# YxZhxn/Ray3D

Measured on AMD Instinct MI355X. Metric: lifted poses/sec (17-joint, 243-frame window), higher is better.
Workload: dtype f32; 1 GPU; BASELINE configs[1]: synthetic 17-joint 243-frame windows, batch 256 per GPU, forward-only pos+trj (C=256, latent 256, stage 3, camera embedding); batch_per_gpu=256, receptive_field=243, joints=17, parallelism=dp1 (independent window batches, no data-path collective), clock_settle_steps=60, world_size_observed=1

## Files before the change

ray3d_amd/csrc/r3d_tiles.hpp:

```cpp
#pragma once
#include <hip/hip_runtime.h>

#include <algorithm>
#include <type_traits>

#include "r3d_internal.hpp"

namespace r3d {

#ifndef R3D_TS
#define R3D_TS 0
#endif
#ifdef R3D_TIMING
#define R3D_TSTAMP(slot) do { if (dbg && threadIdx.x == 0) dbg[slot] = wall_clock64(); } while (0)
#else
#define R3D_TSTAMP(slot) do { } while (0)
#endif

typedef float f32x16 __attribute__((ext_vector_type(16)));
typedef float f32x4 __attribute__((ext_vector_type(4)));

#define R3D_AS1 __attribute__((address_space(1)))
__device__ __forceinline__ f32x4 gload4(const float *p) { return *(const R3D_AS1 f32x4 *)p; }
__device__ __forceinline__ float gload1(const float *p) { return *(const R3D_AS1 float *)p; }
__device__ __forceinline__ void gstore1(float *p, float v) { *(R3D_AS1 float *)p = v; }
constexpr int ACT_AUX = 16;
typedef unsigned u32x4 __attribute__((ext_vector_type(4)));
typedef unsigned R3D_AS1 *gu32;
struct LateWait { int dw, ndep; gu32 cnt, abort_flag; long long spin_ticks; };
__device__ __forceinline__ void wait_deps_reg(const int dw, const int ndep, const gu32 cnt, const gu32 abort_flag, const long long spin_ticks);
__device__ __forceinline__ __amdgpu_buffer_rsrc_t act_rsrc(const float *base) {
    return __builtin_amdgcn_make_buffer_rsrc(const_cast<float *>(base), 0, 0x7fffffff, 0x00020000);
}
__device__ __forceinline__ f32x4 act_load4(__amdgpu_buffer_rsrc_t r, int byte_off) {
    return __builtin_bit_cast(f32x4, __builtin_amdgcn_raw_buffer_load_b128(r, byte_off, 0, ACT_AUX));
}
__device__ __forceinline__ float act_load1(__amdgpu_buffer_rsrc_t r, int byte_off) {
    return __builtin_bit_cast(float, __builtin_amdgcn_raw_buffer_load_b32(r, byte_off, 0, ACT_AUX));
}
__device__ __forceinline__ void act_store4(__amdgpu_buffer_rsrc_t r, int byte_off, f32x4 v) {
    __builtin_amdgcn_raw_buffer_store_b128(__builtin_bit_cast(u32x4, v), r, byte_off, 0, ACT_AUX);
}
__device__ __forceinline__ void act_store1(__amdgpu_buffer_rsrc_t r, int byte_off, float v) {
    __builtin_amdgcn_raw_buffer_store_b32(__builtin_bit_cast(unsigned, v), r, byte_off, 0, ACT_AUX);
}
__device__ __forceinline__ void tile_drain() { asm volatile("s_waitcnt vmcnt(0)" ::: "memory"); }
__device__ __forceinline__ void tile_signal(const gu32 cnt, const int sig_base, const int sig_add, const int units) {
    int t = threadIdx.x;
    asm volatile("" : "+v"(t));
    if (t < units) __hip_atomic_fetch_add(cnt + sig_base + t, (unsigned)sig_add, __ATOMIC_RELAXED, __HIP_MEMORY_SCOPE_AGENT);
}
__device__ __forceinline__ void tile_signal2(const gu32 cnt, const int base0, const int add0, const int base1, const int add1) {
    int t = threadIdx.x;
    asm volatile("" : "+v"(t));
    if (t < 2) __hip_atomic_fetch_add(cnt + (t == 0 ? base0 : base1), (unsigned)(t == 0 ? add0 : add1), __ATOMIC_RELAXED, __HIP_MEMORY_SCOPE_AGENT);
}
__device__ __forceinline__ float lrelu(const float v, const float slope) { return __builtin_fmaxf(v, v * slope); }


constexpr int LDS_LD = BK + 4;
constexpr int GEMM_THREADS = 512;
constexpr int GEMM_BN = 256;
constexpr int GEMM_MAX_MI = 6;
constexpr int GEMM_STAGES = 3;
constexpr int STAGE_FLOATS = GEMM_MAX_MI * 32 * LDS_LD;
constexpr int LUT_LDS_INTS = 1152;
constexpr int RING_LDS_BYTES = GEMM_STAGES * STAGE_FLOATS * 4;
constexpr int GEMM_LDS_BYTES = 157952;
static_assert(GEMM_LDS_BYTES >= RING_LDS_BYTES, "the ring and the intermediate tile share the allocation");

typedef const LaunchArgs __attribute__((address_space(4))) *LaunchArgsPtr;
typedef const GemmProb __attribute__((address_space(4))) &ProbRef;

constexpr int EPI_LD = GEMM_BN + 4;

constexpr unsigned ACT_SENTINEL_BITS = 0x7fc5a1e7u;
__device__ __forceinline__ float act_canon(const float v) {
    return __builtin_bit_cast(unsigned, v) == ACT_SENTINEL_BITS ? __builtin_bit_cast(float, 0x7fc00000u) : v;
}

template <int MI, int KS>
__device__ __forceinline__ void store_tile(ProbRef P, const f32x16 (&acc)[MI], const int row0, const int col0, float *lds,
                                           const bool second = false) {
    constexpr int COLS = GEMM_BN / KS, WN = 8 / KS;
    constexpr int TPR = COLS / 4;
    constexpr int RPP = GEMM_THREADS / TPR;
    int tid = threadIdx.x;
    asm volatile("" : "+v"(tid));
    const int lane = tid & 63, wave = tid >> 6, li = lane & 31, lh = lane >> 5;
    const int M = P.M, N = P.N;
    const float slope = second ? P.slope2 : P.slope;
    const float *res = P.res;
    const bool canon = P.canon != 0;
    const int ldc = P.ldc, ldr = P.ldr;
    const __amdgpu_buffer_rsrc_t crs = act_rsrc(P.c + (size_t)row0 * ldc + col0);
    const __amdgpu_buffer_rsrc_t rrs = act_rsrc(res ? res + (size_t)row0 * ldr + col0 : P.c);
    const bool writer = wave < WN;
    const float bias = writer ? gload1((second ? P.bias2 : P.bias) + col0 + wave * 32 + li) : 0.0f;
    float *wr = lds + (4 * lh) * EPI_LD + wave * 32 + li;
    const int rd_row = tid / TPR, rd_c4 = (tid % TPR) * 4;
    const bool vec = (col0 + COLS <= N);
#pragma unroll
    for (int mi = 0; mi < MI; ++mi) {
        __syncthreads();
        if (writer) {
#pragma unroll
            for (int r = 0; r < 16; ++r) {
                float v = acc[mi][r] + bias;
                wr[((r & 3) + 8 * (r >> 2)) * EPI_LD] = lrelu(v, slope);
            }
        }
        __syncthreads();
#pragma unroll
        for (int j = 0; j < 32 / RPP; ++j) {
            const int lr = rd_row + RPP * j;
            const int row = row0 + mi * 32 + lr;
            if (row >= M) continue;
            f32x4 v = *reinterpret_cast<const f32x4 *>(lds + lr * EPI_LD + rd_c4);
            const int col = col0 + rd_c4;
            const int lrow = mi * 32 + lr;
            if (vec) {
                if (res) v += act_load4(rrs, (lrow * ldr + rd_c4) * 4);
                if (canon) {
#pragma unroll
                    for (int e = 0; e < 4; ++e) v[e] = act_canon(v[e]);
                }
                act_store4(crs, (lrow * ldc + rd_c4) * 4, v);
            } else {
#pragma unroll
                for (int e = 0; e < 4; ++e)
                    if (col + e < N) {
                        const float o = v[e] + (res ? act_load1(rrs, (lrow * ldr + rd_c4 + e) * 4) : 0.0f);
                        act_store1(crs, (lrow * ldc + rd_c4 + e) * 4, canon ? act_canon(o) : o);
                    }
            }
        }
    }
    __syncthreads();
}

constexpr int PAIR_LD = GEMM_BN + 4;
constexpr int PAIR_MAX_MI = 4;
template <int MI, int KS, bool PAIR = false>
__device__ __forceinline__ void gemm_tile(ProbRef P, const int row0, const int col0, float *smem, long long *dbg, const LateWait late = LateWait{0, 0, nullptr, nullptr, 0}) {
    static_assert(!PAIR || (KS == 1 && MI <= PAIR_MAX_MI), "fused pairs are whole tiles of at most 128 rows");
    constexpr int SF = STAGE_FLOATS;
    R3D_TSTAMP(0);
    static_assert(KS == 1 || (KS == 2 && MI <= 2) || (KS == 4 && MI == 1), "split-K tiles are small tiles");
    constexpr int WN = 8 / KS;
    constexpr int VR = KS * MI * 32;
    constexpr int NA = (VR + 63) / 64;
    constexpr bool PRE = MI <= 3;
    constexpr bool WD2 = MI <= 4;
    constexpr int AD = WD2 ? 5 : 4;
    int tid = threadIdx.x;
    asm volatile("" : "+v"(tid));
    const int lane = tid & 63, wave = tid >> 6;
    const int li = lane & 31, lh = lane >> 5;
    const int wn = wave % WN;
    const int wk = wave / WN;
    const int M = P.M, K = P.K;
    const int nk32 = K / BK;
    const int nk = (nk32 + KS - 1) / KS;
    const int srow = tid >> 3, a_kq = (tid & 7) * 4;

    const bool multi = P.kend[0] < K;
    int seg_ld = P.lda[0], seg_k0 = 0, seg_end = P.kend[0], seg_i = 0;
// ... 35 lines not shown
    auto commit_a = [&](int stage, const Staged &R) {
        float *s = stage == 0 ? smem + st_off : stage == 1 ? smem + SF + st_off : smem + 2 * SF + st_off;
        {
#pragma unroll
            for (int i = 0; i < NA; ++i) *reinterpret_cast<f32x4 *>(s + i * 64 * LDS_LD) = R.a[i];
        }
    };

    const int wave_u = __builtin_amdgcn_readfirstlane(wave);
    __amdgpu_buffer_rsrc_t wrsrc = __builtin_amdgcn_make_buffer_rsrc(
        const_cast<float *>(P.w + ((size_t)((col0 >> 5) + wave_u % WN) * nk32 + wave_u / WN) * 1024), 0,
        (nk32 - wave_u / WN) * 4096, 0x00020000);
    const int w_voff = lane * 16;
    f32x4 rb[4], rbn[4], rbn2[4];
    auto load_w = [&](int kt, f32x4 (&dst)[4]) {
#pragma unroll
        for (int q = 0; q < 4; ++q)
            dst[q] = __builtin_bit_cast(f32x4, __builtin_amdgcn_raw_buffer_load_b128(
                wrsrc, w_voff + q * 1024, kt * KS * 4096, 0));
    };

    f32x16 acc[MI];
#pragma unroll
    for (int mi = 0; mi < MI; ++mi)
#pragma unroll
        for (int r = 0; r < 16; ++r) acc[mi][r] = 0.0f;

    const int a_frag = (wk * MI * 32 + li) * LDS_LD + lh * 16;
    f32x4 av0[PRE ? MI : 1];

    const int last = nk - 1;
    load_w(0, rb);
    if (WD2) load_w(1 < last ? 1 : last, rbn);
    if (late.ndep > 0) wait_deps_reg(late.dw, late.ndep, late.cnt, late.abort_flag, late.spin_ticks);
    {
        Staged r0, r1;
        issue_a(0, r0);
        prep_seg(1 < last ? 1 : last);
        issue_a(1 < last ? 1 : last, r1);
        prep_seg(2 < last ? 2 : last);
        issue_a(2 < last ? 2 : last, ra);
        prep_seg(3 < last ? 3 : last);
        issue_a(3 < last ? 3 : last, ra2);
        prep_seg(4 < last ? 4 : last);
        if (WD2) {
            issue_a(4 < last ? 4 : last, ra3);
            prep_seg(5 < last ? 5 : last);
        }
        if (P.kend[0] < BK) {
            const int width = P.kend[0];
#pragma unroll
            for (int i = 0; i < NA; ++i)
#pragma unroll
                for (int e = 0; e < 4; ++e)
                    if (a_kq + e >= width) r0.a[i][e] = 0.0f;
        }
        commit_a(0, r0);
        commit_a(1, r1);
    }
    __syncthreads();
    if (PRE) {
#pragma unroll
        for (int mi = 0; mi < MI; ++mi) av0[mi] = *reinterpret_cast<const f32x4 *>(smem + a_frag + mi * 32 * LDS_LD);
    }
    R3D_TSTAMP(1);
    int st_cur = 0;
    auto k_tile = [&](int kt, f32x4 (&w_use)[4], f32x4 (&w_load)[4], Staged &stg) {
        const int st_next = st_cur == 2 ? 0 : st_cur + 1, st_next2 = st_next == 2 ? 0 : st_next + 1;
        const float *s = smem + st_cur * SF + a_frag;
        const bool active = KS == 1 || kt * KS + wave_u / WN < nk32;
        auto mfma_q = [&](int q) {
            if (!active) return;
            f32x4 av[MI];
#pragma unroll
            for (int mi = 0; mi < MI; ++mi) {
                if (PRE && q == 0) av[mi] = av0[mi];
                else av[mi] = *reinterpret_cast<const f32x4 *>(s + mi * 32 * LDS_LD + q * 4);
            }
#pragma unroll
            for (int kk = 0; kk < 4; ++kk)
#pragma unroll
                for (int mi = 0; mi < MI; ++mi)
                    acc[mi] = __builtin_amdgcn_mfma_f32_32x32x2f32(av[mi][kk], w_use[q][kk], acc[mi], 0, 0, 0);
        };
        constexpr bool INTERLEAVE = MI >= 3;
        if (!INTERLEAVE) {
            commit_a(st_next2, stg);
            load_w(kt + (WD2 ? 2 : 1) < last ? kt + (WD2 ? 2 : 1) : last, w_load);
            issue_a(kt + AD < last ? kt + AD : last, stg);
            prep_seg(kt + AD + 1 < last ? kt + AD + 1 : last);
        }
        mfma_q(0);
        if (INTERLEAVE) {
            commit_a(st_next2, stg);
            load_w(kt + (WD2 ? 2 : 1) < last ? kt + (WD2 ? 2 : 1) : last, w_load);
        }
        mfma_q(1);
        if (INTERLEAVE) {
            issue_a(kt + AD < last ? kt + AD : last, stg);
            prep_seg(kt + AD + 1 < last ? kt + AD + 1 : last);
        }
        mfma_q(2);
        mfma_q(3);
        if (PRE) {
            const float *sn = smem + st_next * SF + a_frag;
#pragma unroll
            for (int mi = 0; mi < MI; ++mi) av0[mi] = *reinterpret_cast<const f32x4 *>(sn + mi * 32 * LDS_LD);
        }
        __syncthreads();
        st_cur = st_next;
    };
    int kt = 0;
    if (WD2) {
        for (; kt + 2 < nk; kt += 3) {
            k_tile(kt, rb, rbn2, ra);
            k_tile(kt + 1, rbn, rb, ra2);
            k_tile(kt + 2, rbn2, rbn, ra3);
        }
        if (kt < nk) {
            k_tile(kt, rb, rbn2, ra);
            if (kt + 1 < nk) k_tile(kt + 1, rbn, rb, ra2);
        }
    } else {
        for (; kt + 1 < nk; kt += 2) {
            k_tile(kt, rb, rbn, ra);
            k_tile(kt + 1, rbn, rb, ra2);
        }
        if (kt < nk) k_tile(kt, rb, rbn, ra);
    }

    R3D_TSTAMP(2);
    if (KS > 1) {
        constexpr int PHASE_FLOATS = WN * MI * 16 * 64;
        float *red = smem + ((wn * MI) * 16) * 64 + lane;
        if (wk > 0) {
            float *mine = red + wk * PHASE_FLOATS;
#pragma unroll
            for (int mi = 0; mi < MI; ++mi)
#pragma unroll
                for (int r = 0; r < 16; ++r) mine[(mi * 16 + r) * 64] = acc[mi][r];
        }
        __syncthreads();
        if (wk == 0) {
#pragma unroll
            for (int ph = 1; ph < KS; ++ph)
#pragma unroll
                for (int mi = 0; mi < MI; ++mi)
#pragma unroll
                    for (int r = 0; r < 16; ++r) acc[mi][r] += red[ph * PHASE_FLOATS + (mi * 16 + r) * 64];
        }
    }
    R3D_TSTAMP(3);
    if constexpr (PAIR) {
        const float slope1 = P.slope;
        const float bias1 = gload1(P.bias + wave * 32 + li);
        __syncthreads();
#pragma unroll
        for (int mi = 0; mi < MI; ++mi) {
            float *wr = smem + (mi * 32 + 4 * lh) * PAIR_LD + wave * 32 + li;
#pragma unroll
            for (int r = 0; r < 16; ++r) {
                const float v = acc[mi][r] + bias1;
                wr[((r & 3) + 8 * (r >> 2)) * PAIR_LD] = lrelu(v, slope1);
            }
        }
        __syncthreads();
        const int nk2 = P.K2 / BK;
        __amdgpu_buffer_rsrc_t w2rsrc = __builtin_amdgcn_make_buffer_rsrc(
            const_cast<float *>(P.w2 + ((size_t)wave_u * nk2) * 1024), 0, nk2 * 4096, 0x00020000);
        auto load_w2 = [&](int kt, f32x4 (&dst)[4]) {
#pragma unroll
            for (int q = 0; q < 4; ++q)
                dst[q] = __builtin_bit_cast(f32x4, __builtin_amdgcn_raw_buffer_load_b128(w2rsrc, w_voff + q * 1024, kt * 4096, 0));
        };
#pragma unroll
        for (int mi = 0; mi < MI; ++mi)
#pragma unroll
            for (int r = 0; r < 16; ++r) acc[mi][r] = 0.0f;
        const float *h_frag = smem + li * PAIR_LD + lh * 16;
        const int last2 = nk2 - 1;
        auto k_tile2 = [&](int kt2, f32x4 (&w_use)[4], f32x4 (&w_load)[4]) {
            load_w2(kt2 + 2 < last2 ? kt2 + 2 : last2, w_load);
            __builtin_amdgcn_sched_barrier(0);
            const float *s = h_frag + kt2 * BK;
#pragma unroll
            for (int q = 0; q < 4; ++q) {
                f32x4 av[MI];
#pragma unroll
                for (int mi = 0; mi < MI; ++mi) av[mi] = *reinterpret_cast<const f32x4 *>(s + mi * 32 * PAIR_LD + q * 4);
#pragma unroll
                for (int kk = 0; kk < 4; ++kk)
#pragma unroll
                    for (int mi = 0; mi < MI; ++mi)
                        acc[mi] = __builtin_amdgcn_mfma_f32_32x32x2f32(av[mi][kk], w_use[q][kk], acc[mi], 0, 0, 0);
            }
        };
        load_w2(0, rb);
        load_w2(1 < last2 ? 1 : last2, rbn);
        int kt2 = 0;
        for (; kt2 + 2 < nk2; kt2 += 3) {
            k_tile2(kt2, rb, rbn2);
            k_tile2(kt2 + 1, rbn, rb);
            k_tile2(kt2 + 2, rbn2, rbn);
        }
        if (kt2 < nk2) {
            k_tile2(kt2, rb, rbn2);
            if (kt2 + 1 < nk2) k_tile2(kt2 + 1, rbn, rb);
        }
        store_tile<MI, 1>(P, acc, row0, col0, smem, true);
    } else {
        store_tile<MI, KS>(P, acc, row0, col0, smem);
    }
    R3D_TSTAMP(4);
}

template <int NB>
__device__ __forceinline__ void gemm_tile_nb(ProbRef P, ProbRef P2, const int row0, const int row0b, const int col0, const int n0, float *smem, long long *dbg,
                                             const LateWait late = LateWait{0, 0, nullptr, nullptr, 0}) {
    static_assert(NB >= 4 && NB <= 7, "NB = 8 is gemm_tile<1, 1>");
    constexpr int SF = STAGE_FLOATS;
    constexpr int NX = NB - 4;
    constexpr int AD = 5;
    R3D_TSTAMP(0);
    int tid = threadIdx.x;
    asm volatile("" : "+v"(tid));
    const int lane = tid & 63, wave = tid >> 6;
    const int li = lane & 31, lh = lane >> 5;
    const int wave_u = __builtin_amdgcn_readfirstlane(wave);
    const bool main_w = wave_u < 4;
    const bool two = n0 < NB;
    ProbRef PA = two && !main_w ? P2 : P;
    const int rowA = two && !main_w ? row0b : row0;
    const int M = PA.M, K = P.K;
    const int nk = K / BK;
    const int srow = tid >> 3, a_kq = (tid & 7) * 4;
    const int xg0 = (wave_u - 4) * NX;
    int s_blk[4], s_q[4];
#pragma unroll
    for (int s = 0; s < 4; ++s) {
        const int sc = s < NX ? s : 0;
        s_blk[s] = main_w ? wave_u : (NX > 0 ? 4 + (xg0 + sc) / 4 : wave_u - 4);
        s_q[s] = main_w ? s : (NX > 0 ? (xg0 + sc) & 3 : 0);
    }
    const bool multi = PA.kend[0] < K;
// ... 11 lines not shown
    auto prep_seg = [&](int kt) {
        if (!multi) return;
        while (kt * BK >= seg_end) {
            ++seg_i;
            seg_k0 = seg_end;
            seg_ld = PA.lda[seg_i];
            seg_end = PA.kend[seg_i];
            open_seg();
        }
    };
    f32x4 ra, ra2, ra3;
    auto issue_a = [&](int kt, f32x4 &R) {
        R = __builtin_bit_cast(f32x4, __builtin_amdgcn_raw_buffer_load_b128(arsrc, a_voff, (kt * BK - seg_k0) * 4, ACT_AUX));
    };
    const int st_off = srow * LDS_LD + a_kq;
    auto commit_a = [&](int stage, const f32x4 &R) {
        float *sp = stage == 0 ? smem + st_off : stage == 1 ? smem + SF + st_off : smem + 2 * SF + st_off;
        *reinterpret_cast<f32x4 *>(sp) = R;
    };
    const __amdgpu_buffer_rsrc_t wrsrc0 = __builtin_amdgcn_make_buffer_rsrc(
        const_cast<float *>(P.w + (size_t)(col0 >> 5) * nk * 1024), 0, NB * nk * 4096, 0x00020000);
    const __amdgpu_buffer_rsrc_t wrsrc1 = __builtin_amdgcn_make_buffer_rsrc(const_cast<float *>(P2.w), 0, NB * nk * 4096, 0x00020000);
    const int w_voff = lane * 16;
    __amdgpu_buffer_rsrc_t wrsrc[4];
    int w_soff[4], a_off[4];
#pragma unroll
    for (int s = 0; s < 4; ++s) {
        const bool second = s_blk[s] >= n0;
        wrsrc[s] = second ? wrsrc1 : wrsrc0;
        w_soff[s] = __builtin_amdgcn_readfirstlane(((second ? s_blk[s] - n0 : s_blk[s]) * nk) * 4096 + s_q[s] * 1024);
        a_off[s] = (second ? 32 * LDS_LD : 0) + li * LDS_LD + lh * 16 + s_q[s] * 4;
    }
    const int last = nk - 1;
    auto k_loop = [&](auto ns_tag, auto nacc_tag, f32x16 *acc, const __amdgpu_buffer_rsrc_t (&wrs)[4]) {
        constexpr int NS = decltype(ns_tag)::value, NACC = decltype(nacc_tag)::value;
        constexpr int NSL = NS > 0 ? NS : 1;
        f32x4 rb[NSL], rbn[NSL], rbn2[NSL];
        auto load_w = [&](int kt, f32x4 (&dst)[NSL]) {
            if (NS == 0) return;
#pragma unroll
            for (int s = 0; s < NSL; ++s)
                dst[s] = __builtin_bit_cast(f32x4, __builtin_amdgcn_raw_buffer_load_b128(wrs[s], w_voff, w_soff[s] + kt * 4096, 0));
        };
        load_w(0, rb);
        load_w(1 < last ? 1 : last, rbn);
        if (late.ndep > 0) wait_deps_reg(late.dw, late.ndep, late.cnt, late.abort_flag, late.spin_ticks);
        {
            f32x4 r0, r1;
            issue_a(0, r0);
            prep_seg(1 < last ? 1 : last);
            issue_a(1 < last ? 1 : last, r1);
            prep_seg(2 < last ? 2 : last);
            issue_a(2 < last ? 2 : last, ra);
            prep_seg(3 < last ? 3 : last);
            issue_a(3 < last ? 3 : last, ra2);
            prep_seg(4 < last ? 4 : last);
            issue_a(4 < last ? 4 : last, ra3);
            prep_seg(5 < last ? 5 : last);
            commit_a(0, r0);
            commit_a(1, r1);
        }
        __syncthreads();
        f32x4 av0 = *reinterpret_cast<const f32x4 *>(smem + a_off[0]);
        R3D_TSTAMP(1);
        int st_cur = 0;
        auto k_tile = [&](int kt, f32x4 (&w_use)[NSL], f32x4 (&w_load)[NSL], f32x4 &stg) {
            const int st_next = st_cur == 2 ? 0 : st_cur + 1, st_next2 = st_next == 2 ? 0 : st_next + 1;
            const float *sp = smem + st_cur * SF;
            commit_a(st_next2, stg);
            load_w(kt + 2 < last ? kt + 2 : last, w_load);
            issue_a(kt + AD < last ? kt + AD : last, stg);
            prep_seg(kt + AD + 1 < last ? kt + AD + 1 : last);
#pragma unroll
            for (int s = 0; s < NS; ++s) {
                const f32x4 av = s == 0 ? av0 : *reinterpret_cast<const f32x4 *>(sp + a_off[s]);
#pragma unroll
                for (int kk = 0; kk < 4; ++kk)
                    acc[s % NACC] = __builtin_amdgcn_mfma_f32_32x32x2f32(av[kk], w_use[s][kk], acc[s % NACC], 0, 0, 0);
            }
            if (NS > 0) av0 = *reinterpret_cast<const f32x4 *>(smem + st_next * SF + a_off[0]);
            __syncthreads();
            st_cur = st_next;
        };
        int kt = 0;
        for (; kt + 2 < nk; kt += 3) {
            k_tile(kt, rb, rbn2, ra);
            k_tile(kt + 1, rbn, rb, ra2);
            k_tile(kt + 2, rbn2, rbn, ra3);
        }
        if (kt < nk) {
            k_tile(kt, rb, rbn2, ra);
            if (kt + 1 < nk) k_tile(kt + 1, rbn, rb, ra2);
        }
    };
    constexpr int PART = 16 * 64;
    f32x16 fin;
    if (main_w) {
        f32x16 acc[1];
#pragma unroll
        for (int r = 0; r < 16; ++r) acc[0][r] = 0.0f;
        const __amdgpu_buffer_rsrc_t wm[4] = {wrsrc[0], wrsrc[0], wrsrc[0], wrsrc[0]};
        k_loop(std::integral_constant<int, 4>{}, std::integral_constant<int, 1>{}, acc, wm);
        fin = acc[0];
        R3D_TSTAMP(2);
        if (NX > 0) __syncthreads();
    } else {
        constexpr int NA_ = NX > 0 ? NX : 1;
        f32x16 acc[NA_];
#pragma unroll
        for (int a = 0; a < NA_; ++a)
#pragma unroll
            for (int r = 0; r < 16; ++r) acc[a][r] = 0.0f;
        k_loop(std::integral_constant<int, NX>{}, std::integral_constant<int, NA_>{}, acc, wrsrc);
        if (NX > 0) {
            float *red = smem + lane;
#pragma unroll
            for (int a = 0; a < NX; ++a)
#pragma unroll
                for (int r = 0; r < 16; ++r) red[(xg0 + a) * PART + r * 64] = acc[a][r];
            __syncthreads();
#pragma unroll
            for (int r = 0; r < 16; ++r) fin[r] = 0.0f;
            if (wave_u < NB) {
                const float *src = red + (wave_u - 4) * 4 * PART;
#pragma unroll
                for (int g = 0; g < 4; ++g)
#pragma unroll
                    for (int r = 0; r < 16; ++r) fin[r] += src[g * PART + r * 64];
            }
        }
    }
    R3D_TSTAMP(3);
    if (two) {
        const bool writer = wave_u < NB, wsecond = wave_u >= n0;
        const float slope = wsecond ? P2.slope : P.slope;
        const float bias = writer ? gload1((wsecond ? P2.bias + (wave_u - n0) * 32 : P.bias + col0 + wave_u * 32) + li) : 0.0f;
        __syncthreads();
        if (writer) {
            float *wr = smem + (4 * lh) * EPI_LD + wave * 32 + li;
#pragma unroll
            for (int r = 0; r < 16; ++r) wr[((r & 3) + 8 * (r >> 2)) * EPI_LD] = lrelu(fin[r] + bias, slope);
        }
        __syncthreads();
        const int lr = (tid >> 3) & 31, c4 = (tid & 7) * 4;
#pragma unroll
        for (int it = 0; it < (NB + 1) / 2; ++it) {
            const int blk = (wave_u >> 2) + 2 * it;
            if (blk >= NB) break;
            const bool second = blk >= n0;
            ProbRef Q = second ? P2 : P;
            const int qrow = second ? row0b : row0, qcol = second ? (blk - n0) * 32 : col0 + blk * 32;
            if (qrow + lr >= Q.M) continue;
            const float *res = Q.res;
            const int ldc = Q.ldc, ldr = Q.ldr;
            const __amdgpu_buffer_rsrc_t crs = act_rsrc(Q.c + (size_t)qrow * ldc + qcol);
            const __amdgpu_buffer_rsrc_t rrs = act_rsrc(res ? res + (size_t)qrow * ldr + qcol : Q.c);
            f32x4 v = *reinterpret_cast<const f32x4 *>(smem + lr * EPI_LD + blk * 32 + c4);
            if (res) v += act_load4(rrs, (lr * ldr + c4) * 4);
            act_store4(crs, (lr * ldc + c4) * 4, v);
        }
        __syncthreads();
    } else
    {
        constexpr int COLS = NB * 32, TPR = COLS / 4;
        const int N = P.N;
        const float slope = P.slope;
        const float *res = P.res;
        const int ldc = P.ldc, ldr = P.ldr;
        const __amdgpu_buffer_rsrc_t crs = act_rsrc(P.c + (size_t)row0 * ldc + col0);
        const __amdgpu_buffer_rsrc_t rrs = act_rsrc(res ? res + (size_t)row0 * ldr + col0 : P.c);
        const bool writer = wave_u < NB;
        const float bias = writer ? gload1(P.bias + col0 + wave * 32 + li) : 0.0f;
        __syncthreads();
        if (writer) {
            float *wr = smem + (4 * lh) * EPI_LD + wave * 32 + li;
#pragma unroll
            for (int r = 0; r < 16; ++r) wr[((r & 3) + 8 * (r >> 2)) * EPI_LD] = lrelu(fin[r] + bias, slope);
        }
        __syncthreads();
        const bool vec = col0 + COLS <= N;
#pragma unroll
        for (int it = 0; it < (32 * TPR + GEMM_THREADS - 1) / GEMM_THREADS; ++it) {
            const int c = tid + it * GEMM_THREADS;
            if (c >= 32 * TPR) break;
            const int lr = c / TPR, c4 = (c % TPR) * 4;
            if (row0 + lr >= M) continue;
            f32x4 v = *reinterpret_cast<const f32x4 *>(smem + lr * EPI_LD + c4);
            if (vec) {
                if (res) v += act_load4(rrs, (lr * ldr + c4) * 4);
                act_store4(crs, (lr * ldc + c4) * 4, v);
            } else {
#pragma unroll
                for (int e = 0; e < 4; ++e)
                    if (col0 + c4 + e < N) act_store1(crs, (lr * ldc + c4 + e) * 4, v[e] + (res ? act_load1(rrs, (lr * ldr + c4 + e) * 4) : 0.0f));
            }
        }
        __syncthreads();
    }
    R3D_TSTAMP(4);
}

typedef __bf16 bf16x8 __attribute__((ext_vector_type(8)));
typedef __bf16 bf16x2 __attribute__((ext_vector_type(2)));
typedef float f32x2 __attribute__((ext_vector_type(2)));
constexpr int B3_LD = 20;

__device__ __forceinline__ unsigned b3_pack(float a, float b) {
    const f32x2 v = {a, b};
    return __builtin_bit_cast(unsigned, __builtin_convertvector(v, bf16x2));
}
__device__ __forceinline__ float b3_lo(unsigned u) { return __builtin_bit_cast(float, u << 16); }
__device__ __forceinline__ float b3_hi(unsigned u) { return __builtin_bit_cast(float, u & 0xffff0000u); }

__device__ __forceinline__ void b3_split8(const f32x4 &a, const f32x4 &b, bf16x8 (&pl)[3]) {
    typedef unsigned u32x4 __attribute__((ext_vector_type(4)));
    const float x[8] = {a[0], a[1], a[2], a[3], b[0], b[1], b[2], b[3]};
    u32x4 p0, p1, p2;
#ifdef R3D_EXP_NOSPLIT_W
#pragma unroll
    for (int i = 0; i < 4; ++i) p0[i] = p1[i] = p2[i] = b3_pack(x[2 * i], x[2 * i + 1]);
    pl[0] = __builtin_bit_cast(bf16x8, p0);
    pl[1] = __builtin_bit_cast(bf16x8, p1);
// ... 1985 lines not shown
        const int col0 = __builtin_amdgcn_readfirstlane(td.z);
        const int ks = __builtin_amdgcn_readfirstlane(td.w);
        int sig_base = 0, sig_add = 0, tflags = 0, sig_base2 = -1;
        LateWait late{0, 0, nullptr, nullptr, 0};
        TileDeps tdep{nullptr, 0, nullptr, nullptr, false, nullptr, 0};
        if constexpr (DEP) {
            const int4 te = make_int4(__builtin_amdgcn_readlane(dw, 4), __builtin_amdgcn_readlane(dw, 5), __builtin_amdgcn_readlane(dw, 6), __builtin_amdgcn_readlane(dw, 7));
            const int ndep = __builtin_amdgcn_readfirstlane(te.x);
            sig_base = __builtin_amdgcn_readfirstlane(te.y);
            sig_add = __builtin_amdgcn_readfirstlane(te.z);
            tflags = __builtin_amdgcn_readfirstlane(te.w);
#ifdef R3D_TIMING
            if (dbg_arg && threadIdx.x == 0) dbg_arg[16384 + (long long)t * 4 + 0] = wall_clock64();
#endif
#ifndef R3D_TIMING
            constexpr bool LATE = !B3 && !ENC;
#else
            constexpr bool LATE = false;
#endif
            const bool wait_here = ndep > 0 && (!NARROW || !tile_is_narrow(ks));
            if (wait_here && !LATE) wait_deps_reg(dw, ndep, cnt, abort_flag, fargs->spin_ticks);
            if (wait_here && LATE) late = LateWait{dw, ndep, cnt, abort_flag, fargs->spin_ticks};
#ifdef R3D_TIMING
            if (dbg_arg && threadIdx.x == 0) dbg_arg[16384 + (long long)t * 4 + 1] = wall_clock64();
#endif
            tdep = TileDeps{tiles + t * TS, NARROW && tile_is_narrow(ks) ? ndep : 0, cnt, abort_flag, NARROW && fargs->poll != 0, nullptr, fargs->spin_ticks};
#ifdef R3D_TIMING
            if (dbg_arg) tdep.tstamp = dbg_arg + 16384 + (long long)t * 4;
#endif
        }
        ProbRef P = DEP ? *((const GemmProb __attribute__((address_space(4))) *)fargs->probs + pi) : args->p[pi];
#ifdef R3D_TIMING
        dbg = dbg_base && t - t0 < 8 ? dbg_base + (t - t0) * 8 : nullptr;
#endif
        bool signalled = false;
        do {
        if constexpr (ENC) {
            (void)ks;
            switch (mi) {
                case 1: enc_tile<1, UV>(P, row0, col0, new_prob, smem, dbg); break;
                case 2: enc_tile<2, UV>(P, row0, col0, new_prob, smem, dbg); break;
                default: enc_tile<3, UV>(P, row0, col0, new_prob, smem, dbg); break;
            }
        } else {
            if (P.w3 != nullptr) {
                int n = 1;
                while (t + n < t1 && __builtin_amdgcn_readfirstlane(tiles[(t + n) * TS].x) == __builtin_amdgcn_readfirstlane(td.x)) ++n;
#ifdef R3D_TIMING
                long long *run_dbg = dbg_base && t - t0 < 8 ? dbg_base + (t - t0) * 8 : nullptr;
#else
                long long *run_dbg = nullptr;
#endif
                const int4 *tl = tiles + t * TS;
                if (CLIP && P.lut == nullptr) {
                  if constexpr (CLIP) {
                    if (mi >= 2) first_level_shared<2>(P, tl, TS, n, smem, cnt, run_dbg);
                    else first_level_shared<1>(P, tl, TS, n, smem, cnt, run_dbg);
                  }
                } else if (B3 && P.wb3 != nullptr) {
                  if constexpr (B3) {
                    if (P.K <= 64) {
                        if (mi >= 2) first_level_taps_b3<2, false, UV>(P, tl, TS, n, new_prob, smem, cnt, run_dbg);
                        else first_level_taps_b3<1, false, UV>(P, tl, TS, n, new_prob, smem, cnt, run_dbg);
                    } else {
                        if (mi >= 2) first_level_taps_b3<2, true, UV>(P, tl, TS, n, new_prob, smem, cnt, run_dbg);
                        else first_level_taps_b3<1, true, UV>(P, tl, TS, n, new_prob, smem, cnt, run_dbg);
// ... 154 lines not shown
```

ray3d_amd/csrc/r3d_timing.cpp:

```cpp
#ifdef R3D_TIMING
#include <algorithm>
#include <cstdio>
#include <cstring>

#include "r3d_internal.hpp"

namespace r3d {

static long long *timing_buf1 = nullptr;

void timing_arm_forward(const Schedule::Fwd &fw, FwdArgs &fa, hipStream_t stream) {
    if (getenv("R3D_TIMING_STAGE")) {
        const size_t tbytes = (16384 + 4 * 65536) * 8;
        if (!timing_buf1) (void)hipMalloc((void **)&timing_buf1, tbytes);
        (void)hipMemsetAsync(timing_buf1, 0, tbytes, stream);
        if (fw.ntiles <= 65536) fa.dbg = timing_buf1;
    }
}

void timing_report_forward(const Plan *pl, const Schedule::Fwd &fw, const FwdArgs &fa, int64_t B, hipStream_t stream) {
    if (fa.dbg) {
        (void)hipStreamSynchronize(stream);
        std::vector<long long> hw(4 * 1024);
        (void)hipMemcpy(hw.data(), timing_buf1 + 1024, hw.size() * 8, hipMemcpyDeviceToHost);
        long long w0 = 1LL << 62, w1 = 0, e0 = 1LL << 62;
        std::vector<double> d;
        for (int w = 0; w < fw.grid && w < 1024; ++w) {
            w0 = std::min(w0, hw[w * 4 + 2]); w1 = std::max(w1, hw[w * 4 + 3]); e0 = std::min(e0, hw[w * 4 + 3]);
            d.push_back((hw[w * 4 + 3] - hw[w * 4 + 2]) / 100.0);
        }
        std::sort(d.begin(), d.end());
        fprintf(stderr, "[timing] forward: first workgroup start -> last end %.2f us; ends spread over %.2f us; busy min %.1f median %.1f max %.1f us\n",
                (w1 - w0) / 100.0, (w1 - e0) / 100.0, d.front(), d[d.size() / 2], d.back());
        if (getenv("R3D_TIMING_ALL"))
            for (int w = 0; w < fw.grid && w < 1024; ++w)
                fprintf(stderr, "[timing-wg] %d start %.2f end %.2f\n", w, (hw[w * 4 + 2] - w0) / 100.0, (hw[w * 4 + 3] - w0) / 100.0);
        if (const char *dump = getenv("R3D_TIMING_DUMP")) {
            std::vector<long long> tt((size_t)fw.ntiles * 4);
            (void)hipMemcpy(tt.data(), timing_buf1 + 16384, tt.size() * 8, hipMemcpyDeviceToHost);
            if (FILE *f = fopen(dump, "w")) {
                for (int i = 0; i < fw.nprob; ++i) {
                    const ProbSpec &q = pl->probs[i];
                    fprintf(f, "P %d %s rows_per_window %d M %lld N %d K %d fused %d\n", i, pl->m[q.model]->layers[q.layer].weight_key.c_str(),
                            q.rows_per_window, (long long)(B * q.rows_per_window), pl->m[q.model]->layers[q.layer].N,
                            pl->m[q.model]->layers[q.layer].Kpad, q.layer3 >= 0 ? 3 : q.layer2 >= 0 ? 2 : 1);
                }
                for (int w = 0; w < fw.grid; ++w)
                    for (int t = fw.h_wgoff[w]; t < fw.h_wgoff[w + 1]; ++t) {
                        const int *d = &fw.h_tiles[(size_t)t * FWD_TILE_INT4 * 4];
                        fprintf(f, "T %d %d %d %d %d %d %d %d %.2f %.2f %.2f %lld %d\n", w, t, d[0] & 0xff, tile_units(d[0]), d[1], d[2], d[3], d[4],
                                tt[(size_t)t * 4] ? (tt[(size_t)t * 4] - w0) / 100.0 : -1.0, tt[(size_t)t * 4 + 1] ? (tt[(size_t)t * 4 + 1] - w0) / 100.0 : -1.0,
                                tt[(size_t)t * 4 + 2] ? (tt[(size_t)t * 4 + 2] - w0) / 100.0 : -1.0, tt[(size_t)t * 4 + 3],
                                tile_src2(d[0]));
                    }
                fclose(f);
            }
        }
    }
}

static long long *timing_buf = nullptr;

bool timing_arm_stage(size_t si, LaunchArgs &la, hipStream_t stream) {
    const char *tstage = getenv("R3D_TIMING_STAGE");
    const bool timed = tstage && (!strcmp(tstage, "all") || atoi(tstage) == (int)si);
    if (timed) {
        if (!timing_buf) (void)hipMalloc((void **)&timing_buf, (1024 + 4 * 1024) * 8 + 65536);
        (void)hipMemsetAsync(timing_buf, 0, (1024 + 4 * 1024) * 8 + 65536, stream);
        la.dbg = timing_buf;
    }
    return timed;
}

void timing_report_stage(size_t si, const StageSchedule &ss, hipStream_t stream) {
    (void)hipStreamSynchronize(stream);
    std::vector<long long> ht(16 * 64);
    (void)hipMemcpy(ht.data(), timing_buf + 6144, ht.size() * 8, hipMemcpyDeviceToHost);
    std::vector<long long> hw(4 * 1024);
    (void)hipMemcpy(hw.data(), timing_buf + 1024, hw.size() * 8, hipMemcpyDeviceToHost);
    long long w0 = 1LL << 62, w1 = 0, s1 = 0, e0 = 1LL << 62;
    for (int w = 0; w < ss.nwg && w < 1024; ++w) {
        w0 = std::min(w0, hw[w * 4 + 2]); s1 = std::max(s1, hw[w * 4 + 2]);
        w1 = std::max(w1, hw[w * 4 + 3]); e0 = std::min(e0, hw[w * 4 + 3]);
    }
    fprintf(stderr, "[timing] launch %zu: first workgroup start -> last end %.2f us; starts spread over %.2f us, ends over %.2f us; "
            "wg 0: start -> first tile entry %.2f us\n", si, (w1 - w0) / 100.0, (s1 - w0) / 100.0, (w1 - e0) / 100.0,
// ... 36 lines not shown
```

Before: 462,000 poses/s.

## Prefetch residual, bias and second-GEMM weights during final K iterations

The GEMM tile loops now peel the final K iteration so that, instead of issuing dead loads, it prefetches the epilogue's residual rows into registers, and for fused pairs the second GEMM's first weight tiles. Bias loads move before the main loop, and the multi-row epilogue double-buffers residual loads one row-block ahead. The aim is to hide epilogue global-load latency behind MFMA work. The cost is extra register pressure and more template and tail-case complexity. Timing instrumentation for per-tile phases is also extended.

New measurement: 465,300 poses/s, median of 6. About the same (+0.7%).

```diff
diff --git a/ray3d_amd/csrc/r3d_tiles.hpp b/ray3d_amd/csrc/r3d_tiles.hpp
--- a/ray3d_amd/csrc/r3d_tiles.hpp
+++ b/ray3d_amd/csrc/r3d_tiles.hpp
@@ -13,6 +13,7 @@
 #endif
 #ifdef R3D_TIMING
 #define R3D_TSTAMP(slot) do { if (dbg && threadIdx.x == 0) dbg[slot] = wall_clock64(); } while (0)
+constexpr long long FWD_PHASE_STAMPS = 16384 + 4 * 65536;
 #else
 #define R3D_TSTAMP(slot) do { } while (0)
 #endif
@@ -79,9 +80,36 @@
     return __builtin_bit_cast(unsigned, v) == ACT_SENTINEL_BITS ? __builtin_bit_cast(float, 0x7fc00000u) : v;
 }
 
-template <int MI, int KS>
+template <int KS>
+struct EpiAhead {
+    static constexpr int NP = 4 / KS;
+    float bias;
+    f32x4 res[NP];
+    __amdgpu_buffer_rsrc_t rrs;
+    int ldr;
+    bool ahead;
+};
+template <int KS>
+__device__ __forceinline__ void epi_open(ProbRef P, const int row0, const int col0, EpiAhead<KS> &E) {
+    const float *res = P.res;
+    E.ldr = P.ldr;
+    E.ahead = res != nullptr && col0 + GEMM_BN / KS <= P.N && P.canon == 0;
+    E.rrs = __builtin_amdgcn_make_buffer_rsrc(const_cast<float *>(E.ahead ? res + (size_t)row0 * E.ldr + col0 : P.c), 0, E.ahead ? 0x7fffffff : 0, 0x00020000);
+}
+template <int KS>
+__device__ __forceinline__ void epi_request(const EpiAhead<KS> &E, f32x4 (&dst)[4 / KS], const int tid, const int mi, const int row0, const int M) {
+    constexpr int TPR = GEMM_BN / KS / 4, RPP = GEMM_THREADS / TPR;
+    const int rd_row = tid / TPR, rd_c4 = (tid % TPR) * 4, lim = M - 1 - row0;
+#pragma unroll
+    for (int j = 0; j < 32 / RPP; ++j) {
+        const int lrow = mi * 32 + rd_row + RPP * j;
+        dst[j] = act_load4(E.rrs, ((lrow < lim ? lrow : lim) * E.ldr + rd_c4) * 4);
+    }
+}
+
+template <int MI, int KS, bool AHEAD = false, bool FIRST = true>
 __device__ __forceinline__ void store_tile(ProbRef P, const f32x16 (&acc)[MI], const int row0, const int col0, float *lds,
-                                           const bool second = false) {
+                                           const bool second = false, const EpiAhead<KS> *pre = nullptr) {
     constexpr int COLS = GEMM_BN / KS, WN = 8 / KS;
     constexpr int TPR = COLS / 4;
     constexpr int RPP = GEMM_THREADS / TPR;
@@ -96,12 +124,25 @@
     const __amdgpu_buffer_rsrc_t crs = act_rsrc(P.c + (size_t)row0 * ldc + col0);
     const __amdgpu_buffer_rsrc_t rrs = act_rsrc(res ? res + (size_t)row0 * ldr + col0 : P.c);
     const bool writer = wave < WN;
-    const float bias = writer ? gload1((second ? P.bias2 : P.bias) + col0 + wave * 32 + li) : 0.0f;
+    float bias;
+    if constexpr (AHEAD) bias = pre->bias;
+    else bias = writer ? gload1((second ? P.bias2 : P.bias) + col0 + wave * 32 + li) : 0.0f;
     float *wr = lds + (4 * lh) * EPI_LD + wave * 32 + li;
     const int rd_row = tid / TPR, rd_c4 = (tid % TPR) * 4;
     const bool vec = (col0 + COLS <= N);
+    const bool ahead = AHEAD && pre->ahead;
+    f32x4 rcur[4 / KS], rnext[4 / KS];
+    if constexpr (AHEAD && FIRST) {
+#pragma unroll
+        for (int j = 0; j < 4 / KS; ++j) rcur[j] = pre->res[j];
+    } else if constexpr (AHEAD) {
+        epi_request<KS>(*pre, rcur, tid, 0, row0, M);
+    }
 #pragma unroll
     for (int mi = 0; mi < MI; ++mi) {
+        if constexpr (AHEAD && MI > 1) {
+            if (mi + 1 < MI) epi_request<KS>(*pre, rnext, tid, mi + 1, row0, M);
+        }
         __syncthreads();
         if (writer) {
 #pragma unroll
@@ -120,7 +161,8 @@
             const int col = col0 + rd_c4;
             const int lrow = mi * 32 + lr;
             if (vec) {
-                if (res) v += act_load4(rrs, (lrow * ldr + rd_c4) * 4);
+                if (AHEAD && ahead) v += rcur[j];
+                else if (res) v += act_load4(rrs, (lrow * ldr + rd_c4) * 4);
                 if (canon) {
 #pragma unroll
                     for (int e = 0; e < 4; ++e) v[e] = act_canon(v[e]);
@@ -133,6 +175,12 @@
                         const float o = v[e] + (res ? act_load1(rrs, (lrow * ldr + rd_c4 + e) * 4) : 0.0f);
                         act_store1(crs, (lrow * ldc + rd_c4 + e) * 4, canon ? act_canon(o) : o);
                     }
+            }
+        }
+        if constexpr (AHEAD && MI > 1) {
+            if (mi + 1 < MI) {
+#pragma unroll
+                for (int j = 0; j < 4 / KS; ++j) rcur[j] = rnext[j];
             }
         }
     }
@@ -234,6 +282,21 @@
     const int last = nk - 1;
     load_w(0, rb);
     if (WD2) load_w(1 < last ? 1 : last, rbn);
+    EpiAhead<KS> epi;
+    epi_open<KS>(P, row0, col0, epi);
+    epi.bias = gload1((PAIR ? P.bias2 : P.bias) + col0 + wn * 32 + li);
+    float bias1 = 0.0f;
+    if constexpr (PAIR) bias1 = gload1(P.bias + wave * 32 + li);
+    const int nk2 = PAIR ? P.K2 / BK : 0;
+    __amdgpu_buffer_rsrc_t w2rsrc = wrsrc;
+    if constexpr (PAIR)
+        w2rsrc = __builtin_amdgcn_make_buffer_rsrc(const_cast<float *>(P.w2 + ((size_t)wave_u * nk2) * 1024), 0, nk2 * 4096, 0x00020000);
+    const int last2 = nk2 - 1;
+    auto load_w2 = [&](int kt, f32x4 (&dst)[4]) {
+#pragma unroll
+        for (int q = 0; q < 4; ++q)
+            dst[q] = __builtin_bit_cast(f32x4, __builtin_amdgcn_raw_buffer_load_b128(w2rsrc, w_voff + q * 1024, kt * 4096, 0));
+    };
     if (late.ndep > 0) wait_deps_reg(late.dw, late.ndep, late.cnt, late.abort_flag, late.spin_ticks);
     {
         Staged r0, r1;
@@ -267,7 +330,20 @@
     }
     R3D_TSTAMP(1);
     int st_cur = 0;
-    auto k_tile = [&](int kt, f32x4 (&w_use)[4], f32x4 (&w_load)[4], Staged &stg) {
+    constexpr int T_NONE = 0, T_LAST = 1, T_PEN2 = 2, T_LAST2 = 3;
+    constexpr bool RES_IN_LOOP = MI <= 5;
+    auto k_tile = [&](int kt, f32x4 (&w_use)[4], f32x4 (&w_load)[4], Staged &stg, auto tail_tag) {
+        constexpr int TAIL = decltype(tail_tag)::value;
+        constexpr bool FINAL = TAIL == T_LAST || TAIL == T_LAST2;
+        auto stage_w = [&]() {
+            if constexpr (TAIL == T_NONE) load_w(kt + (WD2 ? 2 : 1) < last ? kt + (WD2 ? 2 : 1) : last, w_load);
+            else if constexpr (TAIL == T_PEN2) load_w2(0, w_load);
+            else if constexpr (TAIL == T_LAST2) load_w2(1 < last2 ? 1 : last2, w_load);
+            else if constexpr (!PAIR && RES_IN_LOOP) {
+                epi_request<KS>(epi, epi.res, tid, 0, row0, M);
+                __builtin_amdgcn_sched_barrier(0);
+            }
+        };
         const int st_next = st_cur == 2 ? 0 : st_cur + 1, st_next2 = st_next == 2 ? 0 : st_next + 1;
         const float *s = smem + st_cur * SF + a_frag;
         const bool active = KS == 1 || kt * KS + wave_u / WN < nk32;
@@ -287,24 +363,26 @@
         };
         constexpr bool INTERLEAVE = MI >= 3;
         if (!INTERLEAVE) {
-            commit_a(st_next2, stg);
-            load_w(kt + (WD2 ? 2 : 1) < last ? kt + (WD2 ? 2 : 1) : last, w_load);
+            if (!FINAL) commit_a(st_next2, stg);
+            stage_w();
+            if (!FINAL) {
+                issue_a(kt + AD < last ? kt + AD : last, stg);
+                prep_seg(kt + AD + 1 < last ? kt + AD + 1 : last);
+            }
+        }
+        mfma_q(0);
+        if (INTERLEAVE) {
+            if (!FINAL) commit_a(st_next2, stg);
+            stage_w();
+        }
+        mfma_q(1);
+        if (INTERLEAVE && !FINAL) {
             issue_a(kt + AD < last ? kt + AD : last, stg);
             prep_seg(kt + AD + 1 < last ? kt + AD + 1 : last);
         }
-        mfma_q(0);
-        if (INTERLEAVE) {
-            commit_a(st_next2, stg);
-            load_w(kt + (WD2 ? 2 : 1) < last ? kt + (WD2 ? 2 : 1) : last, w_load);
-        }
-        mfma_q(1);
-        if (INTERLEAVE) {
-            issue_a(kt + AD < last ? kt + AD : last, stg);
-            prep_seg(kt + AD + 1 < last ? kt + AD + 1 : last);
-        }
         mfma_q(2);
         mfma_q(3);
-        if (PRE) {
+        if (PRE && !FINAL) {
             const float *sn = smem + st_next * SF + a_frag;
 #pragma unroll
             for (int mi = 0; mi < MI; ++mi) av0[mi] = *reinterpret_cast<const f32x4 *>(sn + mi * 32 * LDS_LD);
@@ -312,23 +390,38 @@
         __syncthreads();
         st_cur = st_next;
     };
+    constexpr std::integral_constant<int, T_NONE> t_none{};
+    constexpr std::integral_constant<int, T_LAST> t_last{};
     int kt = 0;
+    bool w2_ahead = false;
     if (WD2) {
-        for (; kt + 2 < nk; kt += 3) {
-            k_tile(kt, rb, rbn2, ra);
-            k_tile(kt + 1, rbn, rb, ra2);
-            k_tile(kt + 2, rbn2, rbn, ra3);
-        }
-        if (kt < nk) {
-            k_tile(kt, rb, rbn2, ra);
-            if (kt + 1 < nk) k_tile(kt + 1, rbn, rb, ra2);
+        for (; kt + 3 < nk; kt += 3) {
+            k_tile(kt, rb, rbn2, ra, t_none);
+            k_tile(kt + 1, rbn, rb, ra2, t_none);
+            k_tile(kt + 2, rbn2, rbn, ra3, t_none);
+        }
+        if (kt + 1 == nk) {
+            k_tile(kt, rb, rbn2, ra, t_last);
+        } else if (kt + 2 == nk) {
+            k_tile(kt, rb, rbn2, ra, t_none);
+            k_tile(kt + 1, rbn, rb, ra2, t_last);
+        } else {
+            k_tile(kt, rb, rbn2, ra, t_none);
+            k_tile(kt + 1, rbn, rb, ra2, std::integral_constant<int, PAIR ? T_PEN2 : T_NONE>{});
+            k_tile(kt + 2, rbn2, rbn, ra3, std::integral_constant<int, PAIR ? T_LAST2 : T_LAST>{});
+            w2_ahead = PAIR;
         }
     } else {
-        for (; kt + 1 < nk; kt += 2) {
-            k_tile(kt, rb, rbn, ra);
-            k_tile(kt + 1, rbn, rb, ra2);
-        }
-        if (kt < nk) k_tile(kt, rb, rbn, ra);
+        for (; kt + 2 < nk; kt += 2) {
+            k_tile(kt, rb, rbn, ra, t_none);
+            k_tile(kt + 1, rbn, rb, ra2, t_none);
+        }
+        if (kt + 1 == nk) {
+            k_tile(kt, rb, rbn, ra, t_last);
+        } else {
+            k_tile(kt, rb, rbn, ra, t_none);
+            k_tile(kt + 1, rbn, rb, ra2, t_last);
+        }
     }
 
     R3D_TSTAMP(2);
@@ -355,7 +448,6 @@
     R3D_TSTAMP(3);
     if constexpr (PAIR) {
         const float slope1 = P.slope;
-        const float bias1 = gload1(P.bias + wave * 32 + li);
         __syncthreads();
 #pragma unroll
         for (int mi = 0; mi < MI; ++mi) {
@@ -367,22 +459,14 @@
             }
         }
         __syncthreads();
-        const int nk2 = P.K2 / BK;
-        __amdgpu_buffer_rsrc_t w2rsrc = __builtin_amdgcn_make_buffer_rsrc(
-            const_cast<float *>(P.w2 + ((size_t)wave_u * nk2) * 1024), 0, nk2 * 4096, 0x00020000);
-        auto load_w2 = [&](int kt, f32x4 (&dst)[4]) {
-#pragma unroll
-            for (int q = 0; q < 4; ++q)
-                dst[q] = __builtin_bit_cast(f32x4, __builtin_amdgcn_raw_buffer_load_b128(w2rsrc, w_voff + q * 1024, kt * 4096, 0));
-        };
 #pragma unroll
         for (int mi = 0; mi < MI; ++mi)
 #pragma unroll
             for (int r = 0; r < 16; ++r) acc[mi][r] = 0.0f;
         const float *h_frag = smem + li * PAIR_LD + lh * 16;
-        const int last2 = nk2 - 1;
-        auto k_tile2 = [&](int kt2, f32x4 (&w_use)[4], f32x4 (&w_load)[4]) {
-            load_w2(kt2 + 2 < last2 ? kt2 + 2 : last2, w_load);
+        auto k_tile2 = [&](int kt2, f32x4 (&w_use)[4], f32x4 (&w_load)[4], auto tail_tag) {
+            if constexpr (decltype(tail_tag)::value == T_LAST) epi_request<KS>(epi, epi.res, tid, 0, row0, M);
+            else load_w2(kt2 + 2 < last2 ? kt2 + 2 : last2, w_load);
             __builtin_amdgcn_sched_barrier(0);
             const float *s = h_frag + kt2 * BK;
 #pragma unroll
@@ -397,21 +481,30 @@
                         acc[mi] = __builtin_amdgcn_mfma_f32_32x32x2f32(av[mi][kk], w_use[q][kk], acc[mi], 0, 0, 0);
             }
         };
-        load_w2(0, rb);
-        load_w2(1 < last2 ? 1 : last2, rbn);
+        if (!w2_ahead) {
+            load_w2(0, rb);
+            load_w2(1 < last2 ? 1 : last2, rbn);
+        }
         int kt2 = 0;
-        for (; kt2 + 2 < nk2; kt2 += 3) {
-            k_tile2(kt2, rb, rbn2);
-            k_tile2(kt2 + 1, rbn, rb);
-            k_tile2(kt2 + 2, rbn2, rbn);
-        }
-        if (kt2 < nk2) {
-            k_tile2(kt2, rb, rbn2);
-            if (kt2 + 1 < nk2) k_tile2(kt2 + 1, rbn, rb);
-        }
-        store_tile<MI, 1>(P, acc, row0, col0, smem, true);
+        for (; kt2 + 3 < nk2; kt2 += 3) {
+            k_tile2(kt2, rb, rbn2, t_none);
+            k_tile2(kt2 + 1, rbn, rb, t_none);
+            k_tile2(kt2 + 2, rbn2, rbn, t_none);
+        }
+        if (kt2 + 1 == nk2) {
+            k_tile2(kt2, rb, rbn2, t_last);
+        } else if (kt2 + 2 == nk2) {
+            k_tile2(kt2, rb, rbn2, t_none);
+            k_tile2(kt2 + 1, rbn, rb, t_last);
+        } else {
+            k_tile2(kt2, rb, rbn2, t_none);
+            k_tile2(kt2 + 1, rbn, rb, t_none);
+            k_tile2(kt2 + 2, rbn2, rbn, t_last);
+        }
+        R3D_TSTAMP(5);
+        store_tile<MI, 1, true>(P, acc, row0, col0, smem, true, &epi);
     } else {
-        store_tile<MI, KS>(P, acc, row0, col0, smem);
+        store_tile<MI, KS, true, RES_IN_LOOP>(P, acc, row0, col0, smem, false, &epi);
     }
     R3D_TSTAMP(4);
 }
@@ -489,6 +582,46 @@
         a_off[s] = (second ? 32 * LDS_LD : 0) + li * LDS_LD + lh * 16 + s_q[s] * 4;
     }
     const int last = nk - 1;
+    constexpr int NIT = (NB + 1) / 2;
+    static_assert(NIT == (32 * NB * 8 + GEMM_THREADS - 1) / GEMM_THREADS, "both epilogues make NIT passes");
+    const int wb = wave_u < NB ? wave_u : NB - 1;
+    const float *bias_p = (wb >= n0 ? P2.bias + (wb - n0) * 32 : P.bias + col0 + wb * 32) + li;
+    float bias = 0.0f;
+    const bool ahead1 = !two && P.res != nullptr && col0 + NB * 32 <= P.N && P.canon == 0;
+    const int ldr0 = P.ldr, ldr1 = P2.ldr;
+    const bool on0 = two ? P.res != nullptr : ahead1, on1 = two && P2.res != nullptr;
+    const __amdgpu_buffer_rsrc_t rq0 = __builtin_amdgcn_make_buffer_rsrc(
+        const_cast<float *>(on0 ? P.res + (size_t)row0 * ldr0 + col0 : P.c), 0, on0 ? 0x7fffffff : 0, 0x00020000);
+    const __amdgpu_buffer_rsrc_t rq1 = __builtin_amdgcn_make_buffer_rsrc(
+        const_cast<float *>(on1 ? P2.res + (size_t)row0b * ldr1 : P.c), 0, on1 ? 0x7fffffff : 0, 0x00020000);
+    int r_voff[NIT];
+    f32x4 r_pre[NIT];
+    auto blk_of = [&](int it) { const int b = (wave_u >> 2) + 2 * it; return b < NB ? b : NB - 1; };
+    auto open_res = [&]() {
+        const int M0 = P.M, M1 = P2.M;
+#pragma unroll
+        for (int it = 0; it < NIT; ++it) {
+            if (two) {
+                const int blk = blk_of(it), lr = (tid >> 3) & 31, c4 = (tid & 7) * 4;
+                const bool second = blk >= n0;
+                const int lim = second ? M1 - 1 - row0b : M0 - 1 - row0;
+                r_voff[it] = ((lr < lim ? lr : lim) * (second ? ldr1 : ldr0) + (second ? blk - n0 : blk) * 32 + c4) * 4;
+            } else {
+                constexpr int TPR = NB * 8;
+                const int c = tid + it * GEMM_THREADS, cc = c < 32 * TPR ? c : 32 * TPR - 1;
+                const int lr = cc / TPR, c4 = (cc % TPR) * 4, lim = M0 - 1 - row0;
+                r_voff[it] = ((lr < lim ? lr : lim) * ldr0 + c4) * 4;
+            }
+        }
+    };
+    auto request_res = [&]() {
+#pragma unroll
+        for (int it = 0; it < NIT; ++it) {
+            const bool second = blk_of(it) >= n0;
+            r_pre[it] = act_load4(second ? rq1 : rq0, r_voff[it]);
+        }
+        __builtin_amdgcn_sched_barrier(0);
+    };
     auto k_loop = [&](auto ns_tag, auto nacc_tag, f32x16 *acc, const __amdgpu_buffer_rsrc_t (&wrs)[4]) {
         constexpr int NS = decltype(ns_tag)::value, NACC = decltype(nacc_tag)::value;
         constexpr int NSL = NS > 0 ? NS : 1;
@@ -501,6 +634,8 @@
         };
         load_w(0, rb);
         load_w(1 < last ? 1 : last, rbn);
+        bias = gload1(bias_p);
+        open_res();
         if (late.ndep > 0) wait_deps_reg(late.dw, late.ndep, late.cnt, late.abort_flag, late.spin_ticks);
         {
             f32x4 r0, r1;
@@ -521,13 +656,18 @@
         f32x4 av0 = *reinterpret_cast<const f32x4 *>(smem + a_off[0]);
         R3D_TSTAMP(1);
         int st_cur = 0;
-        auto k_tile = [&](int kt, f32x4 (&w_use)[NSL], f32x4 (&w_load)[NSL], f32x4 &stg) {
+        auto k_tile = [&](int kt, f32x4 (&w_use)[NSL], f32x4 (&w_load)[NSL], f32x4 &stg, auto final_tag) {
+            constexpr bool FINAL = decltype(final_tag)::value;
             const int st_next = st_cur == 2 ? 0 : st_cur + 1, st_next2 = st_next == 2 ? 0 : st_next + 1;
             const float *sp = smem + st_cur * SF;
-            commit_a(st_next2, stg);
-            load_w(kt + 2 < last ? kt + 2 : last, w_load);
-            issue_a(kt + AD < last ? kt + AD : last, stg);
-            prep_seg(kt + AD + 1 < last ? kt + AD + 1 : last);
+            if constexpr (FINAL) {
+                request_res();
+            } else {
+                commit_a(st_next2, stg);
+                load_w(kt + 2 < last ? kt + 2 : last, w_load);
+                issue_a(kt + AD < last ? kt + AD : last, stg);
+                prep_seg(kt + AD + 1 < last ? kt + AD + 1 : last);
+            }
 #pragma unroll
             for (int s = 0; s < NS; ++s) {
                 const f32x4 av = s == 0 ? av0 : *reinterpret_cast<const f32x4 *>(sp + a_off[s]);
@@ -535,19 +675,27 @@
                 for (int kk = 0; kk < 4; ++kk)
                     acc[s % NACC] = __builtin_amdgcn_mfma_f32_32x32x2f32(av[kk], w_use[s][kk], acc[s % NACC], 0, 0, 0);
             }
-            if (NS > 0) av0 = *reinterpret_cast<const f32x4 *>(smem + st_next * SF + a_off[0]);
+            if (NS > 0 && !FINAL) av0 = *reinterpret_cast<const f32x4 *>(smem + st_next * SF + a_off[0]);
             __syncthreads();
             st_cur = st_next;
         };
+        constexpr std::false_type t_none{};
+        constexpr std::true_type t_last{};
         int kt = 0;
-        for (; kt + 2 < nk; kt += 3) {
-            k_tile(kt, rb, rbn2, ra);
-            k_tile(kt + 1, rbn, rb, ra2);
-            k_tile(kt + 2, rbn2, rbn, ra3);
-        }
-        if (kt < nk) {
-            k_tile(kt, rb, rbn2, ra);
-            if (kt + 1 < nk) k_tile(kt + 1, rbn, rb, ra2);
+        for (; kt + 3 < nk; kt += 3) {
+            k_tile(kt, rb, rbn2, ra, t_none);
+            k_tile(kt + 1, rbn, rb, ra2, t_none);
+            k_tile(kt + 2, rbn2, rbn, ra3, t_none);
+        }
+        if (kt + 1 == nk) {
+            k_tile(kt, rb, rbn2, ra, t_last);
+        } else if (kt + 2 == nk) {
+            k_tile(kt, rb, rbn2, ra, t_none);
+            k_tile(kt + 1, rbn, rb, ra2, t_last);
+        } else {
+            k_tile(kt, rb, rbn2, ra, t_none);
+            k_tile(kt + 1, rbn, rb, ra2, t_none);
+            k_tile(kt + 2, rbn2, rbn, ra3, t_last);
         }
     };
     constexpr int PART = 16 * 64;
@@ -591,7 +739,6 @@
     if (two) {
         const bool writer = wave_u < NB, wsecond = wave_u >= n0;
         const float slope = wsecond ? P2.slope : P.slope;
-        const float bias = writer ? gload1((wsecond ? P2.bias + (wave_u - n0) * 32 : P.bias + col0 + wave_u * 32) + li) : 0.0f;
         __syncthreads();
         if (writer) {
             float *wr = smem + (4 * lh) * EPI_LD + wave * 32 + li;
@@ -609,11 +756,10 @@
             const int qrow = second ? row0b : row0, qcol = second ? (blk - n0) * 32 : col0 + blk * 32;
             if (qrow + lr >= Q.M) continue;
             const float *res = Q.res;
-            const int ldc = Q.ldc, ldr = Q.ldr;
+            const int ldc = Q.ldc;
             const __amdgpu_buffer_rsrc_t crs = act_rsrc(Q.c + (size_t)qrow * ldc + qcol);
-            const __amdgpu_buffer_rsrc_t rrs = act_rsrc(res ? res + (size_t)qrow * ldr + qcol : Q.c);
             f32x4 v = *reinterpret_cast<const f32x4 *>(smem + lr * EPI_LD + blk * 32 + c4);
-            if (res) v += act_load4(rrs, (lr * ldr + c4) * 4);
+            if (res) v += r_pre[it];
             act_store4(crs, (lr * ldc + c4) * 4, v);
         }
         __syncthreads();
@@ -627,7 +773,6 @@
         const __amdgpu_buffer_rsrc_t crs = act_rsrc(P.c + (size_t)row0 * ldc + col0);
         const __amdgpu_buffer_rsrc_t rrs = act_rsrc(res ? res + (size_t)row0 * ldr + col0 : P.c);
         const bool writer = wave_u < NB;
-        const float bias = writer ? gload1(P.bias + col0 + wave * 32 + li) : 0.0f;
         __syncthreads();
         if (writer) {
             float *wr = smem + (4 * lh) * EPI_LD + wave * 32 + li;
@@ -644,7 +789,8 @@
             if (row0 + lr >= M) continue;
             f32x4 v = *reinterpret_cast<const f32x4 *>(smem + lr * EPI_LD + c4);
             if (vec) {
-                if (res) v += act_load4(rrs, (lr * ldr + c4) * 4);
+                if (ahead1) v += r_pre[it];
+                else if (res) v += act_load4(rrs, (lr * ldr + c4) * 4);
                 act_store4(crs, (lr * ldc + c4) * 4, v);
             } else {
 #pragma unroll
@@ -2696,6 +2842,7 @@
         ProbRef P = DEP ? *((const GemmProb __attribute__((address_space(4))) *)fargs->probs + pi) : args->p[pi];
 #ifdef R3D_TIMING
         dbg = dbg_base && t - t0 < 8 ? dbg_base + (t - t0) * 8 : nullptr;
+        if (DEP && dbg_arg) dbg = dbg_arg + FWD_PHASE_STAMPS + (long long)t * 8;
 #endif
         bool signalled = false;
         do {
diff --git a/ray3d_amd/csrc/r3d_timing.cpp b/ray3d_amd/csrc/r3d_timing.cpp
--- a/ray3d_amd/csrc/r3d_timing.cpp
+++ b/ray3d_amd/csrc/r3d_timing.cpp
@@ -11,7 +11,7 @@
 
 void timing_arm_forward(const Schedule::Fwd &fw, FwdArgs &fa, hipStream_t stream) {
     if (getenv("R3D_TIMING_STAGE")) {
-        const size_t tbytes = (16384 + 4 * 65536) * 8;
+        const size_t tbytes = (16384 + 12 * 65536) * 8;
         if (!timing_buf1) (void)hipMalloc((void **)&timing_buf1, tbytes);
         (void)hipMemsetAsync(timing_buf1, 0, tbytes, stream);
         if (fw.ntiles <= 65536) fa.dbg = timing_buf1;
@@ -36,22 +36,25 @@
             for (int w = 0; w < fw.grid && w < 1024; ++w)
                 fprintf(stderr, "[timing-wg] %d start %.2f end %.2f\n", w, (hw[w * 4 + 2] - w0) / 100.0, (hw[w * 4 + 3] - w0) / 100.0);
         if (const char *dump = getenv("R3D_TIMING_DUMP")) {
-            std::vector<long long> tt((size_t)fw.ntiles * 4);
+            std::vector<long long> tt((size_t)fw.ntiles * 4), ph((size_t)fw.ntiles * 8);
             (void)hipMemcpy(tt.data(), timing_buf1 + 16384, tt.size() * 8, hipMemcpyDeviceToHost);
+            (void)hipMemcpy(ph.data(), timing_buf1 + 16384 + 4 * 65536, ph.size() * 8, hipMemcpyDeviceToHost);
             if (FILE *f = fopen(dump, "w")) {
                 for (int i = 0; i < fw.nprob; ++i) {
                     const ProbSpec &q = pl->probs[i];
-                    fprintf(f, "P %d %s rows_per_window %d M %lld N %d K %d fused %d\n", i, pl->m[q.model]->layers[q.layer].weight_key.c_str(),
+                    fprintf(f, "P %d %s rows_per_window %d M %lld N %d K %d fused %d res %d\n", i, pl->m[q.model]->layers[q.layer].weight_key.c_str(),
                             q.rows_per_window, (long long)(B * q.rows_per_window), pl->m[q.model]->layers[q.layer].N,
-                            pl->m[q.model]->layers[q.layer].Kpad, q.layer3 >= 0 ? 3 : q.layer2 >= 0 ? 2 : 1);
+                            pl->m[q.model]->layers[q.layer].Kpad, q.layer3 >= 0 ? 3 : q.layer2 >= 0 ? 2 : 1, q.res_buf >= 0 ? 1 : 0);
                 }
                 for (int w = 0; w < fw.grid; ++w)
                     for (int t = fw.h_wgoff[w]; t < fw.h_wgoff[w + 1]; ++t) {
                         const int *d = &fw.h_tiles[(size_t)t * FWD_TILE_INT4 * 4];
-                        fprintf(f, "T %d %d %d %d %d %d %d %d %.2f %.2f %.2f %lld %d\n", w, t, d[0] & 0xff, tile_units(d[0]), d[1], d[2], d[3], d[4],
+                        fprintf(f, "T %d %d %d %d %d %d %d %d %.2f %.2f %.2f %lld %d", w, t, d[0] & 0xff, tile_units(d[0]), d[1], d[2], d[3], d[4],
                                 tt[(size_t)t * 4] ? (tt[(size_t)t * 4] - w0) / 100.0 : -1.0, tt[(size_t)t * 4 + 1] ? (tt[(size_t)t * 4 + 1] - w0) / 100.0 : -1.0,
                                 tt[(size_t)t * 4 + 2] ? (tt[(size_t)t * 4 + 2] - w0) / 100.0 : -1.0, tt[(size_t)t * 4 + 3],
                                 tile_src2(d[0]));
+                        for (int s = 0; s < 5; ++s) fprintf(f, " %.2f", ph[(size_t)t * 8 + s] ? (ph[(size_t)t * 8 + s] - w0) / 100.0 : -1.0);
+                        fprintf(f, "\n");
                     }
                 fclose(f);
             }
```
